# MCG-NJU/LinK

Measured on AMD Instinct MI355X. Metric: voxels/s through one LinK (3x7)^3 block, 100k active voxels C=64, higher is better.
Workload: dtype f32

## Files before the change

include/link_amd.h:

```cpp
#ifndef LINK_AMD_H_
#define LINK_AMD_H_

#include <stddef.h>
#include <stdint.h>

#ifdef __cplusplus
extern "C" {
#endif

#define LINK_OK 0
#define LINK_ERR_ARG (-1)
#define LINK_ERR_LAUNCH (-2)
#define LINK_ERR_WORKSPACE (-3)
#define LINK_BATCH_TIMEOUT (-4)

int link_abi_version(void);
int32_t link_abi_struct_size(int32_t which);
const char *link_last_error(void);


int link_hash(const int32_t *coords, int64_t n, int64_t *out, void *stream);

int link_kernel_hash(const int32_t *coords, int64_t n, const int32_t *offsets, int64_t k,
                     int64_t *out, void *stream);
// ... 408 lines not shown
                              void *stream);

typedef struct link_block_ctx link_block_ctx_t;
int link_block_ctx_create(link_block_ctx_t **out);
int link_block_ctx_destroy(link_block_ctx_t *ctx);
int64_t link_pair_plan_arena(int64_t n, int32_t kvol, int32_t skip_centre, int64_t offs[11]);

int link_dc_neighbor_map(const int32_t *coords, int64_t n, const link_dc_grid_t *g , const uint32_t *cnt,
                         const int32_t *slots, int32_t step, int32_t *nbr, void *stream);

#define LINK_BLOCK_DONE 0
#define LINK_BLOCK_MISS 1
typedef struct {
  const link_dc_buffers_t *buf;
  const link_dc_grid_t *g;
  const link_elk_desc_t *desc;
  int64_t n;
  int32_t mean_max, cell_max;
  int32_t ts;
  int32_t subm;
  int32_t *nbr;
  int32_t *pair_arena;
  int64_t pair_arena_words;
  float *contrib;
  int64_t contrib_rows;
  const float *w;
  const void *ws;
  const int32_t *w_big;
  const float *nl_w, *nl_b;
  float nl_eps;
  int32_t flags;
  void *out;
  int32_t bbox[8];
  int32_t stats[4];
  int32_t verdict;
  int32_t reserved;
} link_block_args_t;
int link_elk_block_forward(link_block_ctx_t *ctx, link_block_args_t *args , void *stream);

typedef struct link_dc_batch link_dc_batch_t;
int link_dc_batch_create(link_dc_batch_t **out);
int link_dc_batch_destroy(link_dc_batch_t *ctx);
int link_elk_core_dense_forward_batch(link_dc_batch_t *ctx, const link_dc_buffers_t *frames ,
                                      const int64_t *n , int32_t nframes, const link_dc_grid_t *g ,
                                      const link_elk_desc_t *desc , void *stream);
int link_dc_batch_submit(link_dc_batch_t *ctx, const link_dc_buffers_t *frames , const int64_t *n ,
                         int32_t nframes, const link_dc_grid_t *g , const link_elk_desc_t *desc , void *stream,
                         int64_t *ticket );
int link_dc_batch_join(link_dc_batch_t *ctx, int64_t ticket, void *stream);
int link_dc_batch_status(link_dc_batch_t *ctx, int32_t *out );
int link_dc_batch_set_timing(link_dc_batch_t *ctx, int32_t on);
int link_dc_batch_kernel_times(link_dc_batch_t *ctx, int64_t ticket, float *ms );
int link_dc_batch_set_debug(link_dc_batch_t *ctx, uint64_t *k1_rows, uint64_t *k2_rows);
int link_streams_share_queue(void *stream_a, void *stream_b, double *delay_us );
int link_dc_batch_probe_streams(link_dc_batch_t *ctx, hipStream_t stream, double *delays_us );

#define LINK_NMS_ROTATE 0
#define LINK_NMS_NORMAL 1
#define LINK_NMS_CIRCLE 2
int link_boxes_overlap_bev(const float *boxes_a, int64_t na, const float *boxes_b, int64_t nb, float *out , void *stream);
int link_boxes_iou_bev(const float *boxes_a, int64_t na, const float *boxes_b, int64_t nb, float *out , void *stream);
size_t link_nms_workspace_bytes(int64_t n);
int link_nms_mask(const float *boxes, int64_t cap, const int32_t *n_dev, int32_t pred, float thr, uint64_t *mask, void *stream);
int link_nms_reduce(const uint64_t *mask, int64_t cap, const int32_t *n_dev, int32_t post_max, int64_t *keep ,
                    int32_t *count , void *stream);
int link_nms_bev(const float *boxes, int64_t cap, const int32_t *n_dev, int32_t pred, float thr, int32_t post_max, void *workspace,
                 size_t workspace_bytes, int64_t *keep , int32_t *count , void *stream);
typedef struct {
  float out_size_factor, voxel_size[2], pc_range[2], score_threshold, post_center_range[6];
} link_center_geom_t;
int link_center_decode(const float *hm, const float *reg, const float *height, const float *dim, const float *rot, const float *vel,
                       int32_t batch, int32_t num_cls, int32_t h, int32_t w, const link_center_geom_t *geom , float *boxes,
                       int32_t *labels, float *scores, int32_t *counts, void *stream);

#define LINK_VOXELIZE_HARD 0
#define LINK_VOXELIZE_DYNAMIC 1
typedef struct {
  float lo[3], hi[3], vs[3];
  int32_t grid[3];
  int32_t max_points, max_voxels, ndim, mode;
} link_voxelize_geom_t;
size_t link_voxelize_workspace_bytes(const link_voxelize_geom_t *geom , int64_t n_points_capacity, int32_t batch);
int link_voxelize(const link_voxelize_geom_t *geom , const float *points, const int32_t *point_offsets ,
                  int32_t batch, int64_t n_points_capacity, void *workspace, size_t workspace_bytes, float *voxels ,
                  float *mean, int32_t *coors , int32_t *num_points, int64_t voxel_capacity,
                  int32_t *voxel_offsets , void *stream);

#ifdef __cplusplus
}
#endif
#endif
```

link_amd/_lib.py:

```python
from __future__ import annotations

import ctypes
import os
from ctypes import POINTER, Structure, c_char_p, c_float, c_int, c_int32, c_int64, c_size_t, c_void_p

_HERE = os.path.dirname(os.path.abspath(__file__))
SO_PATH = os.path.join(_HERE, "lib", "liblink_amd.so")

LINK_OK, LINK_ERR_ARG, LINK_ERR_LAUNCH, LINK_ERR_WORKSPACE, LINK_BATCH_TIMEOUT = 0, -1, -2, -3, -4
HDR_M, HDR_STATUS, HDR_NVALID, HDR_STATUS_ACC, HDR_WORDS = 0, 1, 2, 3, 8
OP_COS, OP_SIN, OP_COSX = 0, 1, 2
ELK_LANE_CHANNEL, ELK_NO_PAIR, ELK_FUSED_GATHER, ELK_NO_DENSE_GRID, ELK_TILES = 1, 2, 4, 8, 16
ELK_LEAN_CS, ELK_LEAN_NO_CS, ELK_LEAN_PM, ELK_LEAN_NO_PM = 32, 64, 128, 256
IO_F32, IO_F16, IO_BF16 = 0, 1, 2
ABI_VERSION = 13
DEBUG = os.environ.get("LINK_AMD_DEBUG", "0") not in ("", "0")


class LinkGrid(Structure):
    _fields_ = [("s", c_int32), ("lo", c_int32 * 4), ("dim", c_int32 * 4)]

    @property
    def cells(self) -> int:
        v = 1
# ... 197 lines not shown
    "link_subm_conv_wgrad_split": (c_int, [c_void_p, c_void_p, c_void_p, c_int64, c_int32, c_int32, c_int32, c_int32, c_void_p, c_void_p]),
    "link_subm_conv_wgrad_reduce": (c_int, [c_void_p, c_int32, c_int32, c_int32, c_int32, c_void_p, c_void_p]),
    "link_subm_conv_ln_add_relu": (c_int, [c_void_p, c_void_p, c_void_p, c_void_p, c_int64, c_int32, c_int32, c_int32,
                                           c_void_p, c_void_p, c_float, c_void_p, c_int32, c_void_p, c_void_p]),
    "link_ln_add_relu_forward": (c_int, [c_void_p] * 4 + [c_int64, c_int32, c_float, c_void_p, c_void_p]),
    "link_ln_add_relu_backward": (c_int, [c_void_p] * 4 + [c_int64, c_int32, c_float] + [c_void_p] * 4),
    "link_sum_partials": (c_int, [c_void_p, c_int32, c_void_p, c_int32, c_void_p, c_int32, c_int64, c_void_p,
                                  c_void_p]),
    "link_premix_ln_backward": (c_int, [c_void_p] * 4 + [c_int64, c_int32, ctypes.c_float] + [c_void_p] * 4),
    "link_premix_ln_io": (c_int, [c_void_p, c_int32] + [c_void_p] * 3 + [c_int64, c_int32, c_float, c_void_p, c_void_p]),
    "link_premix_ln_backward_io": (c_int, [c_void_p, c_int32] + [c_void_p] * 3 + [c_int64, c_int32, c_float] + [c_void_p] * 4),
    "link_ln_add_relu_forward_io": (c_int, [c_void_p, c_int32] + [c_void_p] * 3 + [c_int64, c_int32, c_float, c_void_p, c_void_p]),
    "link_ln_add_relu_backward_io": (c_int, [c_void_p] * 3 + [c_int32, c_void_p, c_int64, c_int32, c_float] + [c_void_p] * 4),
    "link_bn_forward_stats_io": (c_int, [c_void_p, c_int32, c_int64, c_int32, c_float, c_float] + [c_void_p] * 10),
    "link_bn_apply_forward_io": (c_int, [c_void_p, c_int32, c_void_p, c_void_p, c_void_p, c_int64, c_int32, c_int32, c_void_p, c_void_p]),
    "link_bn_backward_reduce_io": (c_int, [c_void_p, c_void_p, c_int32, c_void_p, c_void_p, c_int64, c_int32] + [c_void_p] * 6),
    "link_bn_backward_reduce_relu_io": (c_int, [c_void_p, c_void_p, c_int32] + [c_void_p] * 4 + [c_int64, c_int32] + [c_void_p] * 6),
    "link_bn_apply_backward_io": (c_int, [c_void_p, c_void_p, c_int32] + [c_void_p] * 4 + [c_int64, c_int32, c_void_p, c_void_p]),
    "link_elk_mid_partial_rows": (c_int32, []),
    "link_dc_grid_from": (c_int64, [POINTER(LinkGrid), c_int32, POINTER(LinkDcGrid)]),
    "link_dc_premix_insert": (c_int, [c_void_p] * 5 + [c_int64, c_int32, c_float, POINTER(LinkDcGrid), c_int32] +
                              [c_void_p] * 7),
    "link_dc_modsum": (c_int, [c_void_p] * 6 + [POINTER(LinkElkDesc), POINTER(LinkDcGrid), c_int32, c_void_p,
                               c_void_p, c_void_p]),
    "link_dc_gather": (c_int, [c_void_p, c_void_p, POINTER(LinkElkDesc), POINTER(LinkDcGrid), c_void_p, c_void_p]),
    "link_elk_core_dense_forward": (c_int, [POINTER(LinkDcBuffers), POINTER(LinkDcGrid), POINTER(LinkElkDesc),
                                            c_int64, c_int32, c_void_p]),
    "link_elk_core_lean_forward": (c_int, [POINTER(LinkLeanBuffers), POINTER(LinkGrid), POINTER(LinkElkDesc), c_int64, c_int64,
                                           c_int32, c_void_p]),
    "link_dc_index_probe": (c_int, [POINTER(LinkDcBuffers), POINTER(LinkDcGrid), c_int64, c_void_p, c_void_p]),
    "link_dc_index_ids": (c_int, [c_void_p, c_int64, POINTER(LinkDcGrid)] + [c_void_p] * 5),
    "link_dc_index": (c_int, [c_void_p, c_int64, POINTER(LinkDcGrid)] + [c_void_p] * 5),
    "link_dc_premix_modsum": (c_int, [POINTER(LinkDcBuffers), POINTER(LinkDcGrid), POINTER(LinkElkDesc), c_int64,
                                      c_int32, c_void_p]),
    "link_dc_gather_demod": (c_int, [POINTER(LinkDcBuffers), POINTER(LinkDcGrid), POINTER(LinkElkDesc), c_int64, c_void_p]),
    "link_dc_demod": (c_int, [c_void_p] * 8 + [POINTER(LinkElkDesc), POINTER(LinkDcGrid), c_int64, c_void_p, c_int32,
                              c_void_p]),
    "link_block_ctx_create": (c_int, [POINTER(c_void_p)]),
    "link_block_ctx_destroy": (c_int, [c_void_p]),
    "link_pair_plan_arena": (c_int64, [c_int64, c_int32, c_int32, POINTER(c_int64)]),
    "link_dc_neighbor_map": (c_int, [c_void_p, c_int64, POINTER(LinkDcGrid), c_void_p, c_void_p, c_int32, c_void_p, c_void_p]),
    "link_elk_block_forward": (c_int, [c_void_p, POINTER(LinkBlockArgs), c_void_p]),
    "link_dc_batch_create": (c_int, [POINTER(c_void_p)]),
    "link_dc_batch_destroy": (c_int, [c_void_p]),
    "link_elk_core_dense_forward_batch": (c_int, [c_void_p, POINTER(LinkDcBuffers), POINTER(c_int64), c_int32, POINTER(LinkDcGrid),
                                                  POINTER(LinkElkDesc), c_void_p]),
    "link_dc_batch_submit": (c_int, [c_void_p, POINTER(LinkDcBuffers), POINTER(c_int64), c_int32, POINTER(LinkDcGrid),
                                     POINTER(LinkElkDesc), c_void_p, POINTER(c_int64)]),
    "link_dc_batch_join": (c_int, [c_void_p, c_int64, c_void_p]),
    "link_dc_batch_set_timing": (c_int, [c_void_p, c_int32]),
    "link_dc_batch_kernel_times": (c_int, [c_void_p, c_int64, POINTER(c_float)]),
    "link_dc_batch_status": (c_int, [c_void_p, POINTER(c_int32)]),
    "link_dc_batch_set_debug": (c_int, [c_void_p, c_void_p, c_void_p]),
    "link_dc_batch_probe_streams": (c_int, [c_void_p, c_void_p, POINTER(ctypes.c_double)]),
    "link_streams_share_queue": (c_int, [c_void_p, c_void_p, POINTER(ctypes.c_double)]),
    "link_elk_mid_backward": (c_int, [c_void_p] * 9 + [POINTER(LinkGrid), c_void_p, c_void_p, c_void_p,
                                      POINTER(LinkElkDesc), c_int64, c_int64] + [c_void_p] * 5),
    "link_boxes_overlap_bev": (c_int, [c_void_p, c_int64, c_void_p, c_int64, c_void_p, c_void_p]),
    "link_boxes_iou_bev": (c_int, [c_void_p, c_int64, c_void_p, c_int64, c_void_p, c_void_p]),
    "link_nms_workspace_bytes": (c_size_t, [c_int64]),
    "link_nms_mask": (c_int, [c_void_p, c_int64, c_void_p, c_int32, c_float, c_void_p, c_void_p]),
    "link_nms_reduce": (c_int, [c_void_p, c_int64, c_void_p, c_int32, c_void_p, c_void_p, c_void_p]),
    "link_nms_bev": (c_int, [c_void_p, c_int64, c_void_p, c_int32, c_float, c_int32, c_void_p, c_size_t, c_void_p, c_void_p, c_void_p]),
    "link_center_decode": (c_int, [c_void_p] * 6 + [c_int32] * 4 + [POINTER(LinkCenterGeom)] + [c_void_p] * 5),
    "link_voxelize_workspace_bytes": (c_size_t, [POINTER(LinkVoxelizeGeom), c_int64, c_int32]),
    "link_voxelize": (c_int, [POINTER(LinkVoxelizeGeom), c_void_p, c_void_p, c_int32, c_int64, c_void_p, c_size_t] + [c_void_p] * 4 +
                      [c_int64, c_void_p, c_void_p]),
}

_lib = None


class LinkAmdError(RuntimeError):
    pass


def lib() -> ctypes.CDLL:
    global _lib
    if _lib is None:
        if not os.path.exists(SO_PATH):
            raise LinkAmdError(
                f"{SO_PATH} not found: the HIP extension is not built. Run `python link_amd/build.py` "
                "(or __graft_entry__.build()). link_amd has no CPU/PyTorch fallback.")
        handle = ctypes.CDLL(SO_PATH)
        for name, (res, args) in SIGNATURES.items():
            fn = getattr(handle, name)
            fn.restype = res
            fn.argtypes = args
        if handle.link_abi_version() != ABI_VERSION:
            raise LinkAmdError("liblink_amd.so ABI version mismatch; rebuild with link_amd/build.py")
        for which, cls in enumerate((LinkGrid, LinkElkDesc, LinkElkBuffers, LinkDcGrid, LinkDcTuning, LinkDcBuffers, LinkLeanBuffers, LinkBlockArgs,
                                      LinkVoxelizeGeom)):
            if handle.link_abi_struct_size(which) != ctypes.sizeof(cls):
                raise LinkAmdError(f"liblink_amd.so: layout of {cls.__name__} differs from include/link_amd.h "
                                   f"({ctypes.sizeof(cls)} bytes here, {handle.link_abi_struct_size(which)} in the library)")
        _lib = handle
    return _lib


def current_stream_handle() -> int:
    import torch
    try:
        return torch._C._cuda_getCurrentRawStream(torch._C._cuda_getDevice())
    except AttributeError:
        return torch.cuda.current_stream().cuda_stream

# ... 26 lines not shown
```

link_amd/csrc/dense_batch.hip:

```cpp
#define DC_IO 0
#define DC_IO_NS dcb_f32
#include "dense_batch_impl.h"

namespace dcb_f16 { int batch_set_launch(const link::dc_bt_host_t &, const link_dc_buffers_t *, const int64_t *, int, const link_dc_grid_t &, const link_elk_desc_t &); }
namespace dcb_bf16 { int batch_set_launch(const link::dc_bt_host_t &, const link_dc_buffers_t *, const int64_t *, int, const link_dc_grid_t &, const link_elk_desc_t &); }

using namespace link;
using namespace dcb_f32;

static constexpr int BT_RING = 4;
__global__ void k_dc_batch_spin(unsigned long long *stamp, int ticks) {
  const unsigned long long t0 = __builtin_amdgcn_s_memrealtime();
  if (threadIdx.x == 0) *stamp = t0;
  while (__builtin_amdgcn_s_memrealtime() - t0 < (unsigned long long)ticks) __builtin_amdgcn_s_sleep(16);
}
static bool bt_queue_delay_us(hipStream_t x, hipStream_t y, unsigned long long *scratch , hipEvent_t ev, double *us) {
  unsigned long long h[2] = {0, 0};
  *us = 0.0;
  if (hipStreamSynchronize(x) != hipSuccess || hipStreamSynchronize(y) != hipSuccess) return false;
  hipLaunchKernelGGL(k_dc_batch_spin, dim3(1), dim3(64), 0, x, scratch, 15000);
  if (hipEventRecord(ev, x) != hipSuccess) return false;
  hipLaunchKernelGGL(k_dc_batch_spin, dim3(1), dim3(64), 0, y, scratch + 1, 0);
  if (hipStreamSynchronize(x) != hipSuccess || hipStreamSynchronize(y) != hipSuccess ||
      hipMemcpy(h, scratch, sizeof h, hipMemcpyDeviceToHost) != hipSuccess)
// ... 43 lines not shown
    bool bad = bt_share_queue(c->sc, s_, c->probe_scratch, c->probe_ev);
    for (size_t i = 0; i < c->pool.size() && !bad; i++) bad = bt_share_queue(c->pool[i], s_, c->probe_scratch, c->probe_ev);
    (bad ? rejected : c->pool).push_back(s_);
  }
  while (ok && c->pool.size() < 2 && !rejected.empty()) { c->pool.push_back(rejected.back()); rejected.pop_back(); }
  for (hipStream_t s_ : rejected) (void)hipStreamDestroy(s_);
  ok = ok && c->pool.size() >= 2;
  if (ok) { c->ia = 0; c->ib = 1; c->sa = c->pool[0]; c->sb = c->pool[1]; }
  if (dbg_place)
    fprintf(stderr, "link_dc_batch_create: %zu streams on hardware queues of their own, %zu candidates rejected\n",
            c->pool.size(), rejected.size());
  ok = ok && hipMalloc(reinterpret_cast<void **>(&c->sync), sizeof(int32_t) * BT_RING * BT_SYNC_WORDS) == hipSuccess &&
            hipMemset(c->sync, 0, sizeof(int32_t) * BT_RING * BT_SYNC_WORDS) == hipSuccess;
  for (int i = 0; i < BT_RING && ok; i++) {
#ifndef DC_BT_EVENT_FLAGS
#define DC_BT_EVENT_FLAGS (hipEventDisableTiming | hipEventDisableSystemFence)
#endif
    ok = hipEventCreateWithFlags(&c->ev_in[i], DC_BT_EVENT_FLAGS) == hipSuccess && hipEventCreateWithFlags(&c->ev_ms[i], DC_BT_EVENT_FLAGS) == hipSuccess &&
         hipEventCreateWithFlags(&c->ev_a[i], DC_BT_EVENT_FLAGS) == hipSuccess && hipEventCreateWithFlags(&c->ev_c[i], DC_BT_EVENT_FLAGS) == hipSuccess &&
         hipEventCreateWithFlags(&c->ev_out[i], DC_BT_EVENT_FLAGS) == hipSuccess;
    c->used[i] = false;
  }
  c->calls = 0;
  c->dbg1 = c->dbg2 = nullptr;
  if (!ok) { (void)hipGetLastError(); delete c; return LINK_ERR_LAUNCH; }
  *out = c;
  return LINK_OK;
}

extern "C" int link_dc_batch_destroy(link_dc_batch_t *c) {
  if (!c) return LINK_OK;
  (void)hipStreamSynchronize(c->sa); (void)hipStreamSynchronize(c->sb); (void)hipStreamSynchronize(c->sc);
  for (int i = 0; i < BT_RING; i++) {
    (void)hipEventDestroy(c->ev_in[i]); (void)hipEventDestroy(c->ev_ms[i]); (void)hipEventDestroy(c->ev_a[i]); (void)hipEventDestroy(c->ev_c[i]);
    (void)hipEventDestroy(c->ev_out[i]);
  }
  for (int i = 0; i < BT_RING; i++)
    for (int k = 0; k < 3; k++) { if (c->tb[i][k]) (void)hipEventDestroy(c->tb[i][k]); if (c->te[i][k]) (void)hipEventDestroy(c->te[i][k]); }
  (void)hipFree(c->sync);
  (void)hipFree(c->probe_scratch);
  (void)hipEventDestroy(c->probe_ev);
  for (hipStream_t s_ : c->pool) (void)hipStreamDestroy(s_);
  (void)hipStreamDestroy(c->sc);
  delete c;
  return LINK_OK;
}

extern "C" int link_dc_batch_set_debug(link_dc_batch_t *c, uint64_t *k1_rows, uint64_t *k2_rows) {
  if (!c) return LINK_ERR_ARG;
  c->dbg1 = reinterpret_cast<unsigned long long *>(k1_rows);
  c->dbg2 = reinterpret_cast<unsigned long long *>(k2_rows);
  return DC_BT_PROF ? LINK_OK : 1;
}

extern "C" int link_streams_share_queue(void *a, void *b, double *delay_us) {
  if (!delay_us) return LINK_ERR_ARG;
  unsigned long long *st = nullptr;
  hipEvent_t ev;
  if (hipMalloc(reinterpret_cast<void **>(&st), 16) != hipSuccess) return LINK_ERR_LAUNCH;
  if (hipEventCreateWithFlags(&ev, hipEventDisableTiming) != hipSuccess) { (void)hipFree(st); return LINK_ERR_LAUNCH; }
  const bool ok = bt_queue_delay_us(S(a), S(b), st, ev, delay_us);
  (void)hipEventDestroy(ev);
  (void)hipFree(st);
  if (!ok) { (void)hipGetLastError(); return LINK_ERR_LAUNCH; }
  return LINK_OK;
}

extern "C" int link_dc_batch_probe_streams(link_dc_batch_t *c, hipStream_t caller, double *delays_us ) {
  if (!c || !delays_us) return LINK_ERR_ARG;
  unsigned long long *st = nullptr;
  hipEvent_t ev;
  if (hipMalloc(reinterpret_cast<void **>(&st), 16) != hipSuccess) return LINK_ERR_LAUNCH;
  if (hipEventCreateWithFlags(&ev, hipEventDisableTiming) != hipSuccess) { (void)hipFree(st); return LINK_ERR_LAUNCH; }
  hipStream_t xs[12] = {c->sa, c->sa, c->sb, caller, caller, caller, c->sb, c->sc, c->sc, c->sa, c->sb, c->sc},
              ys[12] = {c->sb, c->sc, c->sc, c->sa, c->sb, c->sc, c->sa, c->sa, c->sb, caller, caller, caller};
  bool ok = true;
  for (int i = 0; i < 12; i++) ok = bt_queue_delay_us(xs[i], ys[i], st, ev, &delays_us[i]) && ok;
  (void)hipEventDestroy(ev);
  (void)hipFree(st);
  if (!ok) { (void)hipGetLastError(); return LINK_ERR_LAUNCH; }
  return LINK_OK;
}

extern "C" int link_dc_batch_set_timing(link_dc_batch_t *c, int32_t on) {
  if (!c) return LINK_ERR_ARG;
  c->timing = on != 0;
  return LINK_OK;
}
extern "C" int link_dc_batch_kernel_times(link_dc_batch_t *c, int64_t ticket, float *ms ) {
  if (!c || !ms || ticket < 0 || ticket >= c->calls || c->calls - ticket > BT_RING) return LINK_ERR_ARG;
  const int q = (int)(ticket % BT_RING);
  if (!c->timed[q]) return LINK_ERR_ARG;
  for (int i = 0; i < 3; i++)
    if (hipEventSynchronize(c->te[q][i]) != hipSuccess || hipEventElapsedTime(&ms[i], c->tb[q][i], c->te[q][i]) != hipSuccess) {
      (void)hipGetLastError();
      return LINK_ERR_LAUNCH;
    }
  return LINK_OK;
}

extern "C" int link_dc_batch_status(link_dc_batch_t *c, int32_t *out) {
  if (!c || !out) return LINK_ERR_ARG;
  if (hipStreamSynchronize(c->sa) != hipSuccess || hipStreamSynchronize(c->sb) != hipSuccess || hipStreamSynchronize(c->sc) != hipSuccess)
    return LINK_ERR_LAUNCH;
  out[0] = 0;
  out[1] = (int32_t)c->calls;
// ... 138 lines not shown
```

link_amd/csrc/dense_batch_common.h:

```cpp
#pragma once
#include <hip/hip_runtime.h>
#include <stdint.h>

#include "link_amd.h"

#ifndef DC_BT_MAX
#define DC_BT_MAX 48
#endif
#ifndef DC_BT_TIMEOUT_TICKS
#define DC_BT_TIMEOUT_TICKS 200000000ull
#endif
#ifndef DC_BT_PROF
#define DC_BT_PROF 0
#endif
#ifndef DC_BT_INS_LEAD
#define DC_BT_INS_LEAD 1000
#endif
#ifndef DC_BT_INS_WAVES
#define DC_BT_INS_WAVES 4
#endif
#ifndef DC_BT_RELEASE_FENCE
#define DC_BT_RELEASE_FENCE 0
#endif

namespace link {
__host__ __device__ constexpr int bt_err() { return 0; }
__host__ __device__ constexpr int bt_cursor(int xcd) { return 16 * (1 + xcd); }
__host__ __device__ constexpr int bt_k1cur(int xcd) { return 16 * (9 + xcd); }
__host__ __device__ constexpr int bt_inscur() { return 16 * 17; }
__host__ __device__ constexpr int bt_ins(int f) { return 16 * (18 + 2 * f); }
__host__ __device__ constexpr int bt_k1(int f) { return 16 * (19 + 2 * f); }
constexpr int BT_SYNC_WORDS = 16 * (18 + 2 * DC_BT_MAX);
struct dc_bt_host_t {
  hipStream_t sa, sb, sc;
  int cus;
  int32_t *sync;
  unsigned long long *dbg1, *dbg2;
};
}
```

link_amd/csrc/dense_batch_impl.h:

```cpp
#include <stdlib.h>

#include <type_traits>
#include <vector>

#include "dense_batch_common.h"
#include "dense_gather.h"
#include "dense_io.h"

namespace DC_IO_NS {
using namespace link;

#include "dense_k1_impl.h"
#include "dense_k2_cfg.h"
#include "dense_gather_quad_impl.h"

static_assert(DC_ST_AUX == 16, "the S rows must leave the L2 (sc1) for the in-launch hand-off K1 -> K2");

struct dc_bt_frame_t {
  const void *feats; const int4 *coords; int4 *slots; uint32_t *cnt; int32_t *cell_n; int32_t *vcell; float *S; int32_t *hdr;
  void *out; int64_t n;
};
struct dc_bt_frames_t { dc_bt_frame_t f[DC_BT_MAX]; };
struct dc_bt_par_t {
  const float *w_pre, *pre_ln_w, *pre_ln_b, *w_pos, *ln_w, *ln_b;
  int cg; float eps;
  unsigned long long *dbg1, *dbg2;
};
__device__ __forceinline__ void bt_row(unsigned long long *dbg, unsigned long long r, unsigned long long a, unsigned long long b,
                                       unsigned long long c, unsigned long long d, unsigned long long e, unsigned long long f) {
  if (!DC_BT_PROF || !dbg) return;
  if (r + 1 >= dbg[1]) return;
  unsigned long long *o = dbg + 8 * (r + 1);
  o[0] = a; o[1] = b; o[2] = c; o[3] = d; o[4] = e; o[5] = f; o[6] = 1;
}


template <typename P>
__device__ __forceinline__ bool bt_wait_ge(P sync, int word, int target, const int nap = 8) {
  int ok = 1;
  if ((threadIdx.x & 63) == 0) {
    const unsigned long long t0 = __builtin_amdgcn_s_memrealtime();
    int spins = 0;
    while (__hip_atomic_load(&sync[word], __ATOMIC_RELAXED, __HIP_MEMORY_SCOPE_AGENT) < target) {
      if (nap > 8) __builtin_amdgcn_s_sleep(64); else __builtin_amdgcn_s_sleep(8);
      if ((++spins & 15) == 0) {
        if (__hip_atomic_load(&sync[bt_err()], __ATOMIC_RELAXED, __HIP_MEMORY_SCOPE_AGENT) != 0) { ok = 0; break; }
        if (__builtin_amdgcn_s_memrealtime() - t0 > DC_BT_TIMEOUT_TICKS) {
          __hip_atomic_store(&sync[bt_err()], 1 + word, __ATOMIC_RELAXED, __HIP_MEMORY_SCOPE_AGENT);
          ok = 0;
          break;
        }
      }
    }
  }
  return __builtin_amdgcn_readfirstlane(ok) != 0;
}

struct dc_bt_ins_args_t { dc_bt_frames_t fr; link_dc_grid_t g; int nframes, wpf; int32_t *sync; };
__global__ void __launch_bounds__(64) k_dc_batch_insert(dc_bt_ins_args_t args_by_value) {
  (void)args_by_value;
#if defined(__HIP_DEVICE_COMPILE__)
  typedef const __attribute__((address_space(4))) dc_bt_ins_args_t *args_ptr_t;
  for (;;) {
    args_ptr_t a = (args_ptr_t)__builtin_amdgcn_kernarg_segment_ptr();
    asm volatile("" : "+s"(a));
    int t = 0;
    if (threadIdx.x == 0) t = __hip_atomic_fetch_add(&a->sync[bt_inscur()], 1, __ATOMIC_RELAXED, __HIP_MEMORY_SCOPE_AGENT);
    t = __builtin_amdgcn_readfirstlane(t);
    const int wpf = a->wpf;
    if (t >= a->nframes * wpf) break;
    const int f = t / wpf, j = t - f * wpf;
    if (f >= DC_BT_INS_LEAD && !bt_wait_ge(a->sync, bt_k1(f - DC_BT_INS_LEAD), 1, 64)) break;
    const link_dc_grid_t g = a->g;
    const int n = (int)a->fr.f[f].n;
    const int4 *__restrict__ coords = a->fr.f[f].coords;
    int32_t *__restrict__ vcell = a->fr.f[f].vcell;
    int32_t *__restrict__ hdr = a->fr.f[f].hdr;
    const __amdgpu_buffer_rsrc_t r_slots = dc_rsrc(a->fr.f[f].slots, (uint32_t)((int64_t)g.vp * g.k * 16));
    const __amdgpu_buffer_rsrc_t r_cnt = dc_rsrc(a->fr.f[f].cnt, (uint32_t)(g.vp * 4));
    if (j == 0 && threadIdx.x == 0) hdr[LINK_HDR_NVALID] = n;
    _Pragma("unroll 1") for (int k = 0; k < 4; k++) {
      const int v = (4 * j + k) * 64 + (int)threadIdx.x;
      if (v >= n) break;
      const int4 rc = coords[v];
      const unsigned ux = (unsigned)(floordiv(rc.x, g.s) - g.lo[0]), uy = (unsigned)(floordiv(rc.y, g.s) - g.lo[1]);
      const unsigned uz = (unsigned)(floordiv(rc.z, g.s) - g.lo[2]), ub = (unsigned)(rc.w - g.lo[3]);
// ... 28 lines not shown
  const int per = (nranges + 7) >> 3;
  const int lo = x * per;
  const int mine = (lo + per < nranges ? lo + per : nranges) - lo;
  if (mine <= 0) return;
  const int total = nframes * mine;
  int32_t *cur = &sync[bt_k1cur(x)];
  int t_next = 0;
  if (lane == 0) t_next = __hip_atomic_fetch_add(cur, 1, __ATOMIC_RELAXED, __HIP_MEMORY_SCOPE_AGENT);
  int pend_f = -1;
  int ins_known = -1;
  for (;;) {
    const int t = __builtin_amdgcn_readfirstlane(t_next);
    if (t >= total) break;
    const unsigned long long tp0 = DC_BT_PROF ? __builtin_amdgcn_s_memrealtime() : 0;
    const int f = t / mine, i = lo + (t - f * mine);
    if (lane == 0) t_next = __hip_atomic_fetch_add(cur, 1, __ATOMIC_RELAXED, __HIP_MEMORY_SCOPE_AGENT);
    const dc_bt_frame_t &F = fr.f[f];
    int ins_a = wpf, ins_b = wpf;
    if (lane == 0) {
      if (f > ins_known) ins_a = __hip_atomic_load(&sync[bt_ins(f)], __ATOMIC_RELAXED, __HIP_MEMORY_SCOPE_AGENT);
      if (f + 1 < nframes && f + 1 > ins_known) ins_b = __hip_atomic_load(&sync[bt_ins(f + 1)], __ATOMIC_RELAXED, __HIP_MEMORY_SCOPE_AGENT);
    }
    const int c_begin = i * cpw;
    const int c_end = (c_begin + cpw < Vi) ? c_begin + cpw : Vi;
    int pc_f, nv_f;
    int4 rf0, rf1, rf2, rf3;
    if (f <= ins_known) dc_k1_prefetch<true>(pc_f, nv_f, rf0, rf1, rf2, rf3, g, F.slots, F.cnt, c_begin, c_end, lane);
    asm volatile("s_waitcnt vmcnt(0)" ::: "memory");
    if (pend_f >= 0 && lane == 0) __hip_atomic_fetch_add(&sync[bt_k1(pend_f)], 1, __ATOMIC_RELAXED, __HIP_MEMORY_SCOPE_AGENT);
    pend_f = f;
    if (f > ins_known) {
      if (__builtin_amdgcn_readfirstlane(ins_a) < wpf && !bt_wait_ge(sync, bt_ins(f), wpf)) return;
      ins_known = f;
      dc_k1_prefetch<true>(pc_f, nv_f, rf0, rf1, rf2, rf3, g, F.slots, F.cnt, c_begin, c_end, lane);
    }
    if (f + 1 < nframes && f + 1 > ins_known && __builtin_amdgcn_readfirstlane(ins_b) >= wpf) ins_known = f + 1;
    if (i == 0 && lane == 0) {
      F.hdr[LINK_HDR_STATUS] = __hip_atomic_load(&F.hdr[LINK_HDR_STATUS_ACC], __ATOMIC_RELAXED, __HIP_MEMORY_SCOPE_AGENT);
      __hip_atomic_store(&F.hdr[LINK_HDR_STATUS_ACC], 0, __ATOMIC_RELAXED, __HIP_MEMORY_SCOPE_AGENT);
    }
    const unsigned long long tp1 = DC_BT_PROF ? __builtin_amdgcn_s_memrealtime() : 0;
    dc_k1_range<C, OP, NB, false, true>(smem_raw, F.feats, F.slots, F.cnt, F.cell_n, p.w_pre, 1.0f, p.eps, F.n, g, false, F.S, nullptr,
                                        nullptr, c_begin, c_end, pc_f, nv_f, rf0, rf1, rf2, rf3, w_big, th_slow, i, 0, 0);
    if (DC_BT_PROF && lane == 0) bt_row(p.dbg1, (unsigned long long)f * nranges + i, (unsigned long long)f, (unsigned long long)i, tp0, tp1, __builtin_amdgcn_s_memrealtime(), (unsigned long long)(blockIdx.x * 4 + (tid >> 6)));
  }
  asm volatile("s_waitcnt vmcnt(0)" ::: "memory");
#if DC_BT_RELEASE_FENCE
  __builtin_amdgcn_fence(__ATOMIC_RELEASE, "agent");
  asm volatile("s_waitcnt vmcnt(0)" ::: "memory");
#endif
  if (pend_f >= 0 && lane == 0) __hip_atomic_fetch_add(&sync[bt_k1(pend_f)], 1, __ATOMIC_RELAXED, __HIP_MEMORY_SCOPE_AGENT);
}

struct dc_bt_k2_args_t {
  dc_bt_frames_t fr;
  dc_bt_par_t p;
  link_dc_grid_t g;
  int nframes, txn, tyn, zsplit, nwg, k1_target;
  int32_t *sync;
};

template <int OP, int R>
__global__ void __launch_bounds__(256 + 64 * (DC_K2Q_CW + (DC_K2Q_PMAP ? 1 : 0)), 4) k_dc_batch_k2(dc_bt_k2_args_t args_by_value) {
  (void)args_by_value;
#if defined(__HIP_DEVICE_COMPILE__)
  static_assert(DC_K2Q_PMAP == 1, "the mapper wave draws the items");
  typedef const __attribute__((address_space(4))) dc_bt_k2_args_t *args_ptr_t;
  constexpr unsigned CTL_THREAD = 256 + 64 * DC_K2Q_CW;
  __shared__ int s_ctl[4];
  const int x = (int)(__builtin_amdgcn_s_getreg((4 - 1) << 11 | 0 << 6 | 20) & 7u);
  if (threadIdx.x == CTL_THREAD) {
    args_ptr_t a = (args_ptr_t)__builtin_amdgcn_kernarg_segment_ptr();
    int32_t *sy = a->sync;
    const int per = (a->nwg + 7) >> 3;
    if (DC_BT_PROF)
      bt_row(a->p.dbg2, (unsigned long long)a->nframes * (8 * per) + blockIdx.x, 9999, 0, __builtin_amdgcn_s_memrealtime(), 0, 0, blockIdx.x);
    const int t = __hip_atomic_fetch_add(&sy[bt_cursor(x)], 1, __ATOMIC_RELAXED, __HIP_MEMORY_SCOPE_AGENT);
    s_ctl[2] = __hip_atomic_fetch_add(&sy[bt_cursor(x)], 1, __ATOMIC_RELAXED, __HIP_MEMORY_SCOPE_AGENT);
    s_ctl[3] = x;
    int f = t < a->nframes * per ? t / per : -1;
    if (f >= 0 && !bt_wait_ge(sy, bt_k1(f), a->k1_target)) f = -1;
    s_ctl[0] = f; s_ctl[1] = f >= 0 ? (t - f * per) * 8 + x : 0;
  }
  __syncthreads();
  for (;;) {
    args_ptr_t a = (args_ptr_t)__builtin_amdgcn_kernarg_segment_ptr();
    asm volatile("" : "+s"(a));
    const int f = __builtin_amdgcn_readfirstlane(s_ctl[0]), bid = __builtin_amdgcn_readfirstlane(s_ctl[1]);
    if (f < 0) break;
    const unsigned long long tq0 = DC_BT_PROF ? __builtin_amdgcn_s_memrealtime() : 0;
    __syncthreads();
    {
      const link_dc_grid_t g = a->g;
      unsigned tidx = threadIdx.x;
      asm volatile("" : "+v"(tidx));
      dc_k2q_body<OP, R, false, true>(a->fr.f[f].S, a->fr.f[f].cell_n, a->fr.f[f].slots, a->p.w_pos, nullptr, a->p.ln_w, a->p.ln_b, a->p.cg,
                                      1.0f, a->p.eps, a->fr.f[f].n, g, a->txn, a->tyn, a->zsplit, a->nwg, a->fr.f[f].out, nullptr, bid, tidx);
    }
    if (threadIdx.x == CTL_THREAD) {
      const unsigned long long tq1 = DC_BT_PROF ? __builtin_amdgcn_s_memrealtime() : 0;
      int32_t *sy = a->sync;
      const int per = (a->nwg + 7) >> 3;
      const int t = s_ctl[2], xc = s_ctl[3];
      int fn = t < a->nframes * per ? t / per : -1;
      if (fn >= 0) {
        s_ctl[2] = __hip_atomic_fetch_add(&sy[bt_cursor(xc)], 1, __ATOMIC_RELAXED, __HIP_MEMORY_SCOPE_AGENT);
        if (!bt_wait_ge(sy, bt_k1(fn), a->k1_target)) fn = -1;
      }
      s_ctl[0] = fn; s_ctl[1] = fn >= 0 ? (t - fn * per) * 8 + xc : 0;
      if (DC_BT_PROF) bt_row(a->p.dbg2, (unsigned long long)f * (8 * per) + bid, (unsigned long long)f, (unsigned long long)bid, tq0, tq1, __builtin_amdgcn_s_memrealtime(), (unsigned long long)blockIdx.x);
    }
    __syncthreads();
  }
#endif
}


template <int OP, int R>
static int batch_launch(const dc_bt_host_t &c, const dc_bt_frames_t &fr, const dc_bt_par_t &p, const link_dc_grid_t &g, const link_elk_desc_t &d,
                        int nframes, int64_t nmax, bool strips) {
  using K1 = dc_k1_cfg<64, OP>;
  using KQ = dc_k2q_cfg<OP, R>;
  constexpr int LDS_GRAN = 1280, LDS_GRANS = 128, K1_STATIC = 256, K2_STATIC = 16;
  constexpr int k1_lds = 65 * LDS_GRAN - K1_STATIC;
  constexpr int k2_lds = KQ::LDS_BYTES;
  static_assert(k1_lds >= K1::LDS_BYTES && (k2_lds + K2_STATIC + LDS_GRAN - 1) / LDS_GRAN <= LDS_GRANS - 65, "LDS shaping of the two persistent roles");
  int32_t *sync = c.sync;
  const int64_t vi = (int64_t)g.dim[0] * g.dim[1] * g.dim[2] * g.dim[3];
  const int k1_wgs = c.cus;
  static const int rpw = [] { const char *e = getenv("LINK_DC_BATCH_RPW"); const int v = e ? atoi(e) : 1; return v < 1 ? 1 : (v > 16 ? 16 : v); }();
  int cpw = (int)((vi + (int64_t)k1_wgs * K1::NW * rpw - 1) / ((int64_t)k1_wgs * K1::NW * rpw));
  if (cpw < 1) cpw = 1;
  const int k1_target = (int)((vi + cpw - 1) / cpw);
  const dc_k2q_tiles_t tq = dc_k2q_tiles(g, R, strips);
  static const int zs_env = [] { const char *e = getenv("LINK_DC_BATCH_ZSPLIT"); const int v = e ? atoi(e) : 1; return v < 1 ? 1 : (v > 8 ? 8 : v); }();
  int zsplit = zs_env;
  if (zsplit > g.dim[2]) zsplit = g.dim[2];
  const int64_t nwg = ((int64_t)tq.txn * tq.tyn + tq.nxs + tq.nys) * g.dim[3] * zsplit;
  if (nwg > (1 << 20)) return LINK_ERR_ARG;
  int wpf = (int)((nmax + 255) / 256);
  if (wpf < 1) wpf = 1;
  (void)hipFuncSetAttribute(reinterpret_cast<const void *>(&k_dc_batch_k1<OP, 2>), hipFuncAttributeMaxDynamicSharedMemorySize, k1_lds);
  (void)hipFuncSetAttribute(reinterpret_cast<const void *>(&k_dc_batch_k2<OP, R>), hipFuncAttributeMaxDynamicSharedMemorySize, k2_lds);
  const int ins_wgs = c.cus;
  const dc_bt_ins_args_t a0{fr, g, nframes, wpf, sync};
  hipLaunchKernelGGL(k_dc_batch_insert, dim3((unsigned)ins_wgs * DC_BT_INS_WAVES), dim3(64), 0, c.sc, a0);
  int rc = check_launch("link_elk_core_dense_forward_batch (insert)");
  if (rc != LINK_OK) return rc;
  hipLaunchKernelGGL((k_dc_batch_k1<OP, 2>), dim3((unsigned)k1_wgs), dim3(64 * K1::NW), k1_lds, c.sa, fr, p, g, nframes, cpw, k1_target, wpf, sync);
  rc = check_launch("link_elk_core_dense_forward_batch (K1)");
  if (rc != LINK_OK) return rc;
  const dc_bt_k2_args_t a2{fr, p, g, nframes, tq.txn, tq.tyn, zsplit, (int)nwg, k1_target, sync};
  static_assert(sizeof(dc_bt_k2_args_t) <= 4096, "kernel arguments");
  hipLaunchKernelGGL((k_dc_batch_k2<OP, R>), dim3((unsigned)c.cus), dim3(KQ::THREADS), k2_lds, c.sb, a2);
  return check_launch("link_elk_core_dense_forward_batch (K2)");
}

int batch_set_launch(const dc_bt_host_t &c, const link_dc_buffers_t *frames, const int64_t *n, int nb, const link_dc_grid_t &g,
                     const link_elk_desc_t &d) {
  const link_dc_buffers_t &b0 = frames[0];
  const dc_bt_par_t p{b0.w_pre, b0.pre_ln_w, b0.pre_ln_b, b0.w_pos, b0.ln_w, b0.ln_b, d.cg, d.eps, c.dbg1, c.dbg2};
  dc_bt_frames_t fr{};
  int64_t nmax = 0;
  for (int i = 0; i < nb; i++) {
    const link_dc_buffers_t &b = frames[i];
    fr.f[i] = dc_bt_frame_t{b.feats, reinterpret_cast<const int4 *>(b.coords), reinterpret_cast<int4 *>(b.slots), b.cnt, b.cell_n, b.vcell, b.S,
                            b.hdr, b.out, n[i]};
    nmax = n[i] > nmax ? n[i] : nmax;
  }
  static const bool sq_env = [] { const char *e = getenv("LINK_DC_BATCH_SQUARE_RIM"); return e && atoi(e) != 0; }();
  const bool strips = !(b0.tune.k2_form & 16) && !sq_env;
  if (d.op == LINK_OP_COS) return d.r == 3 ? batch_launch<LINK_OP_COS, 3>(c, fr, p, g, d, nb, nmax, strips) : batch_launch<LINK_OP_COS, 2>(c, fr, p, g, d, nb, nmax, strips);
  return d.r == 3 ? batch_launch<LINK_OP_SIN, 3>(c, fr, p, g, d, nb, nmax, strips) : batch_launch<LINK_OP_SIN, 2>(c, fr, p, g, d, nb, nmax, strips);
}
}
```

link_amd/csrc/dense_gather_quad_impl.h:

```cpp
#pragma once
#ifndef DC_K2_MAP
#define DC_K2_MAP 1
#endif

#ifndef DC_K2Q_CW
#define DC_K2Q_CW 3
#endif
#ifndef DC_K2Q_PMAP
#define DC_K2Q_PMAP 1
#endif
#ifndef DC_K2Q_EARLY
#define DC_K2Q_EARLY 1
#endif
#ifndef DC_K2Q_RIM
#define DC_K2Q_RIM 1
#endif
#ifndef DC_K2Q_FMA
#define DC_K2Q_FMA 1
#endif

template <int OP, int R, int TX_ = 0, int TY_ = 0>
struct dc_k2q_cfg {
  using K2 = dc_k2_cfg<OP, R, TX_, TY_>;
  static constexpr int PAR_OFF = K2::SPLIT_LDS_BYTES;
// ... 442 lines not shown
#pragma unroll
      for (int j = 0; j < 4; j++)
#pragma unroll
        for (int e = 0; e < 4; e++) {
          const float A0 = Av[0][j][e], A1 = Av[1][j][e], cc_ = cs[j & 1][e], ss_ = sn[j & 1][e];
          if (DC_K2Q_FMA) {
            nv[j][e] = fmaf(OP == LINK_OP_SIN ? -A1 : A1, ss_, A0 * cc_);
          } else {
            if (OP == LINK_OP_SIN) nv[j][e] = __fsub_rn(__fmul_rn(A0, cc_), __fmul_rn(A1, ss_));
            else nv[j][e] = __fadd_rn(__fmul_rn(A0, cc_), __fmul_rn(A1, ss_));
          }
          s += nv[j][e];
        }
      v4f_t gwb[2][4];
      if (DC_K2Q_OVERLAP) lds_rd8_b128_nowait(par, par + 256u, gwb);
      s = dc_quad_sum(s);
      const float mean = s * (1.0f / C);
      float qq = 0.f;
#pragma unroll
      for (int j = 0; j < 4; j++)
#pragma unroll
        for (int e = 0; e < 4; e++) {
          const float d = nv[j][e] - mean;
          qq += d * d;
        }
      qq = dc_quad_sum(qq);
      const float rs = __builtin_amdgcn_rsqf(qq * (1.0f / C) + eps);
      if (DC_K2Q_OVERLAP) lds_wait_pieces(gwb); else lds_rd8_b128(par, par + 256u, gwb);
#pragma unroll
      for (int j = 0; j < 4; j++) {
        float4 o;
        o.x = (nv[j][0] - mean) * rs * gwb[0][j][0] + gwb[1][j][0]; o.y = (nv[j][1] - mean) * rs * gwb[0][j][1] + gwb[1][j][1];
        o.z = (nv[j][2] - mean) * rs * gwb[0][j][2] + gwb[1][j][2]; o.w = (nv[j][3] - mean) * rs * gwb[0][j][3] + gwb[1][j][3];
        io_st4(r_out, (uint32_t)rec.w * (uint32_t)C + (uint32_t)(16 * j + 4 * q), valid, o);
      }
    }
    if (dbg) tq_work += DC_NOW() - tqa;
  }
  if (dbg && lane == 0) {
    unsigned long long *d = dbg + ((size_t)L * 8 + (tidx >> 6)) * 8;
    d[0] = DC_NOW() - tq0; d[1] = tq0; d[2] = tq_bar; d[3] = 0; d[4] = tq_work; d[5] = tq_rounds; d[6] = nplanes; d[7] = 2;
  }
}

struct dc_k2q_tiles_t { int txn, tyn, nxs, nys; };
static inline dc_k2q_tiles_t dc_k2q_tiles(const link_dc_grid_t &g, int r, bool strips) {
  const bool sx = strips && r == 3 && (g.dim[0] & 3) == 1, sy = strips && r == 3 && (g.dim[1] & 3) == 1;
  const int dxs = g.dim[0] - (sx ? 1 : 0), dys = g.dim[1] - (sy ? 1 : 0);
  return dc_k2q_tiles_t{(dxs + 3) / 4, (dys + 3) / 4, sx ? (g.dim[1] + DC_K2Q_STRIP - 1) / DC_K2Q_STRIP : 0,
                        sy ? (dxs + DC_K2Q_STRIP - 1) / DC_K2Q_STRIP : 0};
}

template <int OP, int R, bool DIV, bool COH = false>
__device__ __forceinline__ void dc_k2q_body(
    const float *__restrict__ S_, const int32_t *__restrict__ cell_n, const int4 *__restrict__ slots,
    const float *__restrict__ w_pos, const float *__restrict__ alpha, const float *__restrict__ ln_w,
    const float *__restrict__ ln_b, int cg, float coord_div, float eps, int64_t n, const link_dc_grid_t &g, int txn, int tyn,
    int zsplit, int nwg, void *__restrict__ out, unsigned long long *__restrict__ dbg, const int bid, const unsigned tidx) {
  using KS = typename dc_k2_cfg<OP, R>::G;
  const int per = (nwg + 7) >> 3;
  const int L = (bid & 7) * per + (bid >> 3);
  if (L >= nwg) return;
  int t = L;
  const int zseg = t % zsplit; t /= zsplit;
  const bool sx = txn * KS::TX < g.dim[0], sy = tyn * KS::TY < g.dim[1];
  const int per_b = txn * tyn;
  const int nsq = per_b * g.dim[3];
  if (R != 3 || t < nsq) {
#if DC_K2_MAP
    const int b = t / per_b;
    int tt2 = t - b * per_b;
    const int H = (tyn + 1) >> 1;
    int tx, ty;
    if (tt2 < txn * H) { tx = tt2 / H; ty = tt2 - tx * H; }
    else { tt2 -= txn * H; const int H2 = tyn - H; tx = tt2 / H2; ty = H + tt2 - tx * H2; }
#else
    const int ty = t % tyn; t /= tyn;
    const int tx = t % txn;
    const int b = t / txn;
#endif
    dc_k2q_tile<OP, R, DIV, COH, 0>(S_, cell_n, slots, w_pos, alpha, ln_w, ln_b, cg, coord_div, eps, n, g, b, tx * KS::TX, ty * KS::TY, zseg, zsplit,
                                    out, dbg, L, tidx);
    return;
  }
  if constexpr (R == 3) {
    const int dxs = g.dim[0] - (sx ? 1 : 0);
    const int nxs = sx ? (g.dim[1] + DC_K2Q_STRIP - 1) / DC_K2Q_STRIP : 0, nys = sy ? (dxs + DC_K2Q_STRIP - 1) / DC_K2Q_STRIP : 0;
    int u = t - nsq;
    const int b = u / (nxs + nys);
    u -= b * (nxs + nys);
    if (u < nxs)
      dc_k2q_tile<OP, R, DIV, COH, 1>(S_, cell_n, slots, w_pos, alpha, ln_w, ln_b, cg, coord_div, eps, n, g, b, g.dim[0] - 1, u * DC_K2Q_STRIP,
                                      zseg, zsplit, out, dbg, L, tidx);
    else
      dc_k2q_tile<OP, R, DIV, COH, 2>(S_, cell_n, slots, w_pos, alpha, ln_w, ln_b, cg, coord_div, eps, n, g, b, (u - nxs) * DC_K2Q_STRIP,
                                      g.dim[1] - 1, zseg, zsplit, out, dbg, L, tidx);
  }
}

template <int OP, int R, bool DIV>
__global__ void __launch_bounds__(256 + 64 * (DC_K2Q_CW + (DC_K2Q_PMAP ? 1 : 0)), 4) k_dc_gather_demod_quad(
    const float *__restrict__ S_, const int32_t *__restrict__ cell_n, const int4 *__restrict__ slots,
    const float *__restrict__ w_pos, const float *__restrict__ alpha, const float *__restrict__ ln_w,
    const float *__restrict__ ln_b, int cg, float coord_div, float eps, int64_t n, link_dc_grid_t g, int txn, int tyn,
    int zsplit, int nwg, void *__restrict__ out, unsigned long long *__restrict__ dbg) {
  dc_k2q_body<OP, R, DIV>(S_, cell_n, slots, w_pos, alpha, ln_w, ln_b, cg, coord_div, eps, n, g, txn, tyn, zsplit, nwg, out, dbg,
                          (int)blockIdx.x, threadIdx.x);
}
```

Baseline: 3.152 billion.

## Rotate per-XCD K2 tile slabs across frames in batched persistent scheduler

```diff
diff --git a/include/link_amd.h b/include/link_amd.h
--- a/include/link_amd.h
+++ b/include/link_amd.h
@@ -484,6 +484,9 @@
 int link_dc_batch_set_timing(link_dc_batch_t *ctx, int32_t on);
 int link_dc_batch_kernel_times(link_dc_batch_t *ctx, int64_t ticket, float *ms );
 int link_dc_batch_set_debug(link_dc_batch_t *ctx, uint64_t *k1_rows, uint64_t *k2_rows);
+int link_dc_batch_k2_deal(int32_t nwg, int32_t nframes, int32_t xcd, int32_t mode, int64_t t0, int64_t count, int32_t *frame ,
+                          int32_t *tile );
+int link_dc_batch_k2_deal_mode(void);
 int link_streams_share_queue(void *stream_a, void *stream_b, double *delay_us );
 int link_dc_batch_probe_streams(link_dc_batch_t *ctx, hipStream_t stream, double *delays_us );
 
diff --git a/link_amd/_lib.py b/link_amd/_lib.py
--- a/link_amd/_lib.py
+++ b/link_amd/_lib.py
@@ -273,6 +273,8 @@
     "link_dc_batch_kernel_times": (c_int, [c_void_p, c_int64, POINTER(c_float)]),
     "link_dc_batch_status": (c_int, [c_void_p, POINTER(c_int32)]),
     "link_dc_batch_set_debug": (c_int, [c_void_p, c_void_p, c_void_p]),
+    "link_dc_batch_k2_deal": (c_int, [c_int32, c_int32, c_int32, c_int32, c_int64, c_int64, POINTER(c_int32), POINTER(c_int32)]),
+    "link_dc_batch_k2_deal_mode": (c_int, []),
     "link_dc_batch_probe_streams": (c_int, [c_void_p, c_void_p, POINTER(ctypes.c_double)]),
     "link_streams_share_queue": (c_int, [c_void_p, c_void_p, POINTER(ctypes.c_double)]),
     "link_elk_mid_backward": (c_int, [c_void_p] * 9 + [POINTER(LinkGrid), c_void_p, c_void_p, c_void_p,
diff --git a/link_amd/csrc/dense_batch.hip b/link_amd/csrc/dense_batch.hip
--- a/link_amd/csrc/dense_batch.hip
+++ b/link_amd/csrc/dense_batch.hip
@@ -119,6 +119,26 @@
   c->dbg2 = reinterpret_cast<unsigned long long *>(k2_rows);
   return DC_BT_PROF ? LINK_OK : 1;
 }
+
+extern "C" int link_dc_batch_k2_deal(int32_t nwg, int32_t nframes, int32_t xcd, int32_t mode, int64_t t0, int64_t count, int32_t *frame,
+                                     int32_t *tile) {
+  if (nwg < 1 || nwg > (1 << 20) || nframes < 1 || nframes > DC_BT_MAX || xcd < 0 || xcd > 7 || (mode != 0 && mode != 1) || t0 < 0 || count < 0 ||
+      (count > 0 && (!frame || !tile)))
+    return LINK_ERR_ARG;
+  for (int64_t i = 0; i < count; i++) {
+    const int64_t t = t0 + i;
+    const dc_bt_item_t it = t < (1LL << 31) ? dc_bt_k2_deal(nwg, nframes, xcd, (int)t, mode) : dc_bt_item_t{-1, 0};
+    frame[i] = it.frame;
+    tile[i] = it.tile;
+  }
+  return LINK_OK;
+}
+
+int link::dc_bt_k2_deal_mode() {
+  static const int mode = [] { const char *e = getenv("LINK_DC_BATCH_DEAL"); return e && strcmp(e, "0") == 0 ? 0 : 1; }();
+  return mode;
+}
+extern "C" int link_dc_batch_k2_deal_mode(void) { return link::dc_bt_k2_deal_mode(); }
 
 extern "C" int link_streams_share_queue(void *a, void *b, double *delay_us) {
   if (!delay_us) return LINK_ERR_ARG;
diff --git a/link_amd/csrc/dense_batch_common.h b/link_amd/csrc/dense_batch_common.h
--- a/link_amd/csrc/dense_batch_common.h
+++ b/link_amd/csrc/dense_batch_common.h
@@ -37,4 +37,5 @@
   int32_t *sync;
   unsigned long long *dbg1, *dbg2;
 };
+int dc_bt_k2_deal_mode();
 }
diff --git a/link_amd/csrc/dense_batch_deal.h b/link_amd/csrc/dense_batch_deal.h
--- /dev/null
+++ b/link_amd/csrc/dense_batch_deal.h
@@ -0,0 +1,40 @@
+#pragma once
+#include <hip/hip_runtime.h>
+
+namespace link {
+struct dc_bt_item_t { int frame, tile; };
+
+__host__ __device__ inline void dc_bt_k2_slab(int nwg, int k, int mode, int &start, int &size) {
+  if (mode) {
+    const int base = nwg >> 3, rem = nwg & 7;
+    start = k * base + (k < rem ? k : rem);
+    size = base + (k < rem ? 1 : 0);
+  } else {
+    const int per = (nwg + 7) >> 3;
+    start = k * per;
+    size = nwg - start < per ? nwg - start : per;
+    if (size < 0) size = 0;
+  }
+}
+
+__host__ __device__ inline dc_bt_item_t dc_bt_k2_deal(int nwg, int nframes, int x, int t, int mode) {
+  const dc_bt_item_t past{-1, 0};
+  if (nwg <= 0 || nframes <= 0 || t < 0) return past;
+  x &= 7;
+  int start = 0, size = 0;
+  if (!mode) dc_bt_k2_slab(nwg, x, 0, start, size);
+  const int cyc = mode ? nwg : 8 * size;
+  if (cyc <= 0) return past;
+  const int c = t / cyc;
+  int u = t - c * cyc;
+  if (c >= (nframes + 7) >> 3) return past;
+  for (int i = 0; i < 8; i++) {
+    const int f = 8 * c + i;
+    if (f >= nframes) return past;
+    dc_bt_k2_slab(nwg, mode ? (x + f) & 7 : x, mode, start, size);
+    if (u < size) return dc_bt_item_t{f, start + u};
+    u -= size;
+  }
+  return past;
+}
+}
diff --git a/link_amd/csrc/dense_batch_impl.h b/link_amd/csrc/dense_batch_impl.h
--- a/link_amd/csrc/dense_batch_impl.h
+++ b/link_amd/csrc/dense_batch_impl.h
@@ -1,9 +1,11 @@
 #include <stdlib.h>
+#include <string.h>
 
 #include <type_traits>
 #include <vector>
 
 #include "dense_batch_common.h"
+#include "dense_batch_deal.h"
 #include "dense_gather.h"
 #include "dense_io.h"
 
@@ -27,11 +29,12 @@
   unsigned long long *dbg1, *dbg2;
 };
 __device__ __forceinline__ void bt_row(unsigned long long *dbg, unsigned long long r, unsigned long long a, unsigned long long b,
-                                       unsigned long long c, unsigned long long d, unsigned long long e, unsigned long long f) {
+                                       unsigned long long c, unsigned long long d, unsigned long long e, unsigned long long f,
+                                       unsigned long long xcd = 0) {
   if (!DC_BT_PROF || !dbg) return;
   if (r + 1 >= dbg[1]) return;
   unsigned long long *o = dbg + 8 * (r + 1);
-  o[0] = a; o[1] = b; o[2] = c; o[3] = d; o[4] = e; o[5] = f; o[6] = 1;
+  o[0] = a; o[1] = b; o[2] = c; o[3] = d; o[4] = e; o[5] = f; o[6] = 1; o[7] = xcd;
 }
 
 
@@ -166,11 +169,16 @@
   if (pend_f >= 0 && lane == 0) __hip_atomic_fetch_add(&sync[bt_k1(pend_f)], 1, __ATOMIC_RELAXED, __HIP_MEMORY_SCOPE_AGENT);
 }
 
+__device__ __forceinline__ dc_bt_item_t bt_k2_item(int nwg, int nframes, int x, int t, int mode) {
+  return dc_bt_k2_deal(nwg, nframes, __builtin_amdgcn_readfirstlane(x), __builtin_amdgcn_readfirstlane(t), mode);
+}
+
 struct dc_bt_k2_args_t {
   dc_bt_frames_t fr;
   dc_bt_par_t p;
   link_dc_grid_t g;
   int nframes, txn, tyn, zsplit, nwg, k1_target;
+  int deal;
   int32_t *sync;
 };
 
@@ -182,47 +190,43 @@
   typedef const __attribute__((address_space(4))) dc_bt_k2_args_t *args_ptr_t;
   constexpr unsigned CTL_THREAD = 256 + 64 * DC_K2Q_CW;
   __shared__ int s_ctl[4];
-  const int x = (int)(__builtin_amdgcn_s_getreg((4 - 1) << 11 | 0 << 6 | 20) & 7u);
   if (threadIdx.x == CTL_THREAD) {
     args_ptr_t a = (args_ptr_t)__builtin_amdgcn_kernarg_segment_ptr();
-    int32_t *sy = a->sync;
-    const int per = (a->nwg + 7) >> 3;
+    const int x = (int)(__builtin_amdgcn_s_getreg((4 - 1) << 11 | 0 << 6 | 20) & 7u);
     if (DC_BT_PROF)
-      bt_row(a->p.dbg2, (unsigned long long)a->nframes * (8 * per) + blockIdx.x, 9999, 0, __builtin_amdgcn_s_memrealtime(), 0, 0, blockIdx.x);
-    const int t = __hip_atomic_fetch_add(&sy[bt_cursor(x)], 1, __ATOMIC_RELAXED, __HIP_MEMORY_SCOPE_AGENT);
-    s_ctl[2] = __hip_atomic_fetch_add(&sy[bt_cursor(x)], 1, __ATOMIC_RELAXED, __HIP_MEMORY_SCOPE_AGENT);
+      bt_row(a->p.dbg2, (unsigned long long)a->nframes * a->nwg + blockIdx.x, 9999, 0, __builtin_amdgcn_s_memrealtime(), 0, 0, blockIdx.x, x);
+    s_ctl[0] = -2; s_ctl[1] = 0;
+    s_ctl[2] = __hip_atomic_fetch_add(&a->sync[bt_cursor(x)], 1, __ATOMIC_RELAXED, __HIP_MEMORY_SCOPE_AGENT);
     s_ctl[3] = x;
-    int f = t < a->nframes * per ? t / per : -1;
-    if (f >= 0 && !bt_wait_ge(sy, bt_k1(f), a->k1_target)) f = -1;
-    s_ctl[0] = f; s_ctl[1] = f >= 0 ? (t - f * per) * 8 + x : 0;
   }
   __syncthreads();
   for (;;) {
     args_ptr_t a = (args_ptr_t)__builtin_amdgcn_kernarg_segment_ptr();
     asm volatile("" : "+s"(a));
-    const int f = __builtin_amdgcn_readfirstlane(s_ctl[0]), bid = __builtin_amdgcn_readfirstlane(s_ctl[1]);
-    if (f < 0) break;
+    const int f = __builtin_amdgcn_readfirstlane(s_ctl[0]), L = __builtin_amdgcn_readfirstlane(s_ctl[1]);
+    if (f == -1) break;
     const unsigned long long tq0 = DC_BT_PROF ? __builtin_amdgcn_s_memrealtime() : 0;
     __syncthreads();
-    {
+    if (f >= 0) {
       const link_dc_grid_t g = a->g;
       unsigned tidx = threadIdx.x;
       asm volatile("" : "+v"(tidx));
-      dc_k2q_body<OP, R, false, true>(a->fr.f[f].S, a->fr.f[f].cell_n, a->fr.f[f].slots, a->p.w_pos, nullptr, a->p.ln_w, a->p.ln_b, a->p.cg,
-                                      1.0f, a->p.eps, a->fr.f[f].n, g, a->txn, a->tyn, a->zsplit, a->nwg, a->fr.f[f].out, nullptr, bid, tidx);
+      dc_k2q_tile_of<OP, R, false, true>(a->fr.f[f].S, a->fr.f[f].cell_n, a->fr.f[f].slots, a->p.w_pos, nullptr, a->p.ln_w, a->p.ln_b, a->p.cg,
+                                         1.0f, a->p.eps, a->fr.f[f].n, g, a->txn, a->tyn, a->zsplit, a->fr.f[f].out, nullptr, L, tidx);
     }
     if (threadIdx.x == CTL_THREAD) {
       const unsigned long long tq1 = DC_BT_PROF ? __builtin_amdgcn_s_memrealtime() : 0;
       int32_t *sy = a->sync;
-      const int per = (a->nwg + 7) >> 3;
       const int t = s_ctl[2], xc = s_ctl[3];
-      int fn = t < a->nframes * per ? t / per : -1;
+      const dc_bt_item_t it = bt_k2_item(a->nwg, a->nframes, xc, t, a->deal);
+      int fn = it.frame;
       if (fn >= 0) {
         s_ctl[2] = __hip_atomic_fetch_add(&sy[bt_cursor(xc)], 1, __ATOMIC_RELAXED, __HIP_MEMORY_SCOPE_AGENT);
         if (!bt_wait_ge(sy, bt_k1(fn), a->k1_target)) fn = -1;
       }
-      s_ctl[0] = fn; s_ctl[1] = fn >= 0 ? (t - fn * per) * 8 + xc : 0;
-      if (DC_BT_PROF) bt_row(a->p.dbg2, (unsigned long long)f * (8 * per) + bid, (unsigned long long)f, (unsigned long long)bid, tq0, tq1, __builtin_amdgcn_s_memrealtime(), (unsigned long long)blockIdx.x);
+      s_ctl[0] = fn; s_ctl[1] = it.tile;
+      if (DC_BT_PROF && f >= 0)
+        bt_row(a->p.dbg2, (unsigned long long)f * a->nwg + L, (unsigned long long)f, (unsigned long long)L, tq0, tq1, __builtin_amdgcn_s_memrealtime(), (unsigned long long)blockIdx.x, (unsigned long long)xc);
     }
     __syncthreads();
   }
@@ -264,7 +268,8 @@
   hipLaunchKernelGGL((k_dc_batch_k1<OP, 2>), dim3((unsigned)k1_wgs), dim3(64 * K1::NW), k1_lds, c.sa, fr, p, g, nframes, cpw, k1_target, wpf, sync);
   rc = check_launch("link_elk_core_dense_forward_batch (K1)");
   if (rc != LINK_OK) return rc;
-  const dc_bt_k2_args_t a2{fr, p, g, nframes, tq.txn, tq.tyn, zsplit, (int)nwg, k1_target, sync};
+  const int deal = dc_bt_k2_deal_mode();
+  const dc_bt_k2_args_t a2{fr, p, g, nframes, tq.txn, tq.tyn, zsplit, (int)nwg, k1_target, deal, sync};
   static_assert(sizeof(dc_bt_k2_args_t) <= 4096, "kernel arguments");
   hipLaunchKernelGGL((k_dc_batch_k2<OP, R>), dim3((unsigned)c.cus), dim3(KQ::THREADS), k2_lds, c.sb, a2);
   return check_launch("link_elk_core_dense_forward_batch (K2)");
diff --git a/link_amd/csrc/dense_gather_quad_impl.h b/link_amd/csrc/dense_gather_quad_impl.h
--- a/link_amd/csrc/dense_gather_quad_impl.h
+++ b/link_amd/csrc/dense_gather_quad_impl.h
@@ -518,15 +518,12 @@
 }
 
 template <int OP, int R, bool DIV, bool COH = false>
-__device__ __forceinline__ void dc_k2q_body(
+__device__ __forceinline__ void dc_k2q_tile_of(
     const float *__restrict__ S_, const int32_t *__restrict__ cell_n, const int4 *__restrict__ slots,
     const float *__restrict__ w_pos, const float *__restrict__ alpha, const float *__restrict__ ln_w,
     const float *__restrict__ ln_b, int cg, float coord_div, float eps, int64_t n, const link_dc_grid_t &g, int txn, int tyn,
-    int zsplit, int nwg, void *__restrict__ out, unsigned long long *__restrict__ dbg, const int bid, const unsigned tidx) {
+    int zsplit, void *__restrict__ out, unsigned long long *__restrict__ dbg, const int L, const unsigned tidx) {
   using KS = typename dc_k2_cfg<OP, R>::G;
-  const int per = (nwg + 7) >> 3;
-  const int L = (bid & 7) * per + (bid >> 3);
-  if (L >= nwg) return;
   int t = L;
   const int zseg = t % zsplit; t /= zsplit;
   const bool sx = txn * KS::TX < g.dim[0], sy = tyn * KS::TY < g.dim[1];
@@ -564,6 +561,18 @@
   }
 }
 
+template <int OP, int R, bool DIV, bool COH = false>
+__device__ __forceinline__ void dc_k2q_body(
+    const float *__restrict__ S_, const int32_t *__restrict__ cell_n, const int4 *__restrict__ slots,
+    const float *__restrict__ w_pos, const float *__restrict__ alpha, const float *__restrict__ ln_w,
+    const float *__restrict__ ln_b, int cg, float coord_div, float eps, int64_t n, const link_dc_grid_t &g, int txn, int tyn,
+    int zsplit, int nwg, void *__restrict__ out, unsigned long long *__restrict__ dbg, const int bid, const unsigned tidx) {
+  const int per = (nwg + 7) >> 3;
+  const int L = (bid & 7) * per + (bid >> 3);
+  if (L >= nwg) return;
+  dc_k2q_tile_of<OP, R, DIV, COH>(S_, cell_n, slots, w_pos, alpha, ln_w, ln_b, cg, coord_div, eps, n, g, txn, tyn, zsplit, out, dbg, L, tidx);
+}
+
 template <int OP, int R, bool DIV>
 __global__ void __launch_bounds__(256 + 64 * (DC_K2Q_CW + (DC_K2Q_PMAP ? 1 : 0)), 4) k_dc_gather_demod_quad(
     const float *__restrict__ S_, const int32_t *__restrict__ cell_n, const int4 *__restrict__ slots,
```

Result: faster. 3.230 billion, median of 6 (+2.5%).
